# CICE-Consortium/CICE

Hardware: AMD Instinct MI355X
Metric: EVP subcycle cell-updates/sec (gx1 fp64) (higher is better)
Workload: dtype f64

## Files before the change

### cice_amd/csrc/evp_cell.inc

```

struct StressIn {
    double u_ij, u_im, u_jm, u_mm;
    double v_ij, v_im, v_jm, v_mm;
    double dxT, dyT, dxhy, dyhx, cxp, cyp, cxm, cym, DminTarea, strength;
};

__device__ __forceinline__ void metrics_cell(double hte, double hte_im, double htn, double htn_jm,
                                             double deltaminEVP, StressIn &a)
{
    a.cyp = (c1p5 * hte - p5 * hte_im);
    a.cxp = (c1p5 * htn - p5 * htn_jm);
    a.cym = -(c1p5 * hte_im - p5 * hte);
    a.cxm = -(c1p5 * htn_jm - p5 * htn);
    a.dxhy = p5 * (hte - hte_im);
    a.dyhx = p5 * (htn - htn_jm);
    const double tarea = a.dxT * a.dyT;
    a.DminTarea = deltaminEVP * tarea;
}

template <int CAP, bool SIMPLE = false, bool CORE = false>
__device__ __forceinline__ void visc_replpress(const EvpScalars &p, double strength, double DminArea,
                                               double Delta, double &zetax2, double &etax2,
                                               double &rep_prs)
{
// ... 216 lines not shown
    const double strm_x = KX * (p333 * (M0 + M1) + p166 * (M2 + M3));
    X = strp_x + strm_x + str12x + dxhy * (-csigp + csigm) + dyhx * csig12;
    const double strp_y = KYP * (p333 * (P0 + P3) + p166 * (P1 + P2));
    const double strm_y = -KYP * (p333 * (M0 + M3) + p166 * (M1 + M2));
    Y = strp_y + strm_y + str12y - dyhx * (csigp + csigm) + dxhy * csig12;
}

struct StepuIn {
    double uold, vold;
    double vrelfac;
    double uocn, vocn, waterx, watery, forcex, forcey, Umassdti, fm, uarear, TbU;
    double uvel_init, vvel_init;
    double sx0, sx1, sx2, sx3;
    double sy0, sy1, sy2, sy3;
};

struct StepuOut {
    double u, v, strintx, strinty, taubx, tauby;
};

struct StepuPre {
    double taux, tauy, Cb, cca, ccb, ab2;
    double bu, bv;
};

template <bool SIMPLE = false, bool TBU = true, bool WITH_B = true, class POL = evp_range::LibMath>
__device__ __forceinline__ void stepu_pre_cell(const EvpScalars &p, const StepuIn &a, StepuPre &w, const POL &pol = POL())
{
    const double uold = a.uold, vold = a.vold;
    const double du = a.uocn - uold, dv = a.vocn - vold;
    double vrel;
    if constexpr (POL::ranged) {
        const double speed2 = du * du + dv * dv;
        if (pol.wave_inside(evp_range::outside(evp_range::off_pos(speed2)), false)) vrel = a.vrelfac * evp_range::sqrt_core(speed2);
        else vrel = a.vrelfac * sqrt(speed2);
    } else {
    vrel = a.vrelfac * sqrt(du * du + dv * dv);
    }
    w.taux = vrel * a.waterx;
    w.tauy = vrel * a.watery;
    double Cb = 0.0;
    if (TBU) Cb = a.TbU / (sqrt(uold * uold + vold * vold) + p.u0);
    w.Cb = Cb;
    double cca, ccb;
    if (SIMPLE) {
        cca = p.brlx * a.Umassdti + vrel + Cb;
        ccb = a.fm;
    } else {
        cca = (p.brlx + p.revp) * a.Umassdti + vrel * p.cosw + Cb;
        ccb = a.fm + copysign(1.0, a.fm) * vrel * p.sinw;
    }
    w.cca = cca; w.ccb = ccb;
    w.ab2 = cca * cca + ccb * ccb;
    if (!WITH_B) return;
    if (SIMPLE) {
        w.bu = p.brlx * uold + 0.0;
        w.bv = p.brlx * vold + 0.0;
    } else {
        w.bu = p.brlx * uold + p.revp * a.uvel_init;
        w.bv = p.brlx * vold + p.revp * a.vvel_init;
    }
}

template <bool SIMPLE = false, bool WITH_B = true, class POL = evp_range::LibMath>
__device__ __forceinline__ void stepu_post_cell(const EvpScalars &p, const StepuIn &a, const StepuPre &w, StepuOut &o)
{
    o.strintx = a.uarear * (a.sx0 + a.sx1 + a.sx2 + a.sx3);
    o.strinty = a.uarear * (a.sy0 + a.sy1 + a.sy2 + a.sy3);
    double cc1, cc2;
    if (WITH_B) {
        cc1 = o.strintx + a.forcex + w.taux + a.Umassdti * w.bu;
        cc2 = o.strinty + a.forcey + w.tauy + a.Umassdti * w.bv;
    } else if (SIMPLE) {
        cc1 = o.strintx + a.forcex + w.taux + a.Umassdti * (p.brlx * a.uold + 0.0);
        cc2 = o.strinty + a.forcey + w.tauy + a.Umassdti * (p.brlx * a.vold + 0.0);
    } else {
        cc1 = o.strintx + a.forcex + w.taux + a.Umassdti * (p.brlx * a.uold + p.revp * a.uvel_init);
        cc2 = o.strinty + a.forcey + w.tauy + a.Umassdti * (p.brlx * a.vold + p.revp * a.vvel_init);
    }
    o.u = (w.cca * cc1 + w.ccb * cc2) / w.ab2;
    o.v = (w.cca * cc2 - w.ccb * cc1) / w.ab2;
    if (POL::lazy_taub) return;
    o.taubx = -o.u * w.Cb;
    o.tauby = -o.v * w.Cb;
}

template <bool SIMPLE = false, bool TBU = true, class POL = evp_range::LibMath>
__device__ __forceinline__ void stepu_cell(const EvpScalars &p, const StepuIn &a, StepuOut &o, const POL &pol = POL())
{
    StepuPre w;
    stepu_pre_cell<SIMPLE, TBU, false, POL>(p, a, w, pol);
    stepu_post_cell<SIMPLE, false>(p, a, w, o);
}

struct DeformOut {
    double divu, shear, vort, rdg_conv, rdg_shear;
};

__device__ __forceinline__ void deform_cell(const EvpScalars &p, const StressIn &a, double tarear,
                                            double dyU_ij, double dyU_im, double dyU_jm, double dyU_mm,
                                            double dxU_ij, double dxU_im, double dxU_jm, double dxU_mm,
                                            DeformOut &o)
{
    const double divune = a.cyp * a.u_ij - a.dyT * a.u_im + a.cxp * a.v_ij - a.dxT * a.v_jm;
// ... 41 lines not shown
```

### cice_amd/csrc/evp_device.h

```cpp
#pragma once
const char *evp_env_test(const char *key);
#include <hip/hip_runtime.h>
#include <stdint.h>
#include <algorithm>

struct EvpScalars {
    double arlx1i, denom1, brlx, revp;
    double e_factor, epp2i;
    double capping, Ktens;
    double u0, cosw, sinw;
    double rhow;
};

struct EvpArgs {
    EvpScalars p;
    int nx, ny;
    size_t plane;
    int gx, gy, ntiles;
    int xcdmap;
    const int *tile_list;
    int tile_count;
    int last;
    const int4 *blk;
    const uint8_t *mask;
// ... 41 lines not shown
    const uint8_t *uperm;
    const uint8_t *late_waves;
    const uint8_t *nact;
    const uint8_t *nlate;
    int *cuload;
    unsigned long long *prof;
    int dbg;
    int par0;
    const int2 *rimg;
    void *const *peer_rec;
    const size_t *peer_rstride;
    unsigned long long timeout_ticks;
    const int *seam;
    int tfold;
    const int *img3;
    void *rec_raw[2];
    const int2 *rraw;
    void *const *peer_raw;
    const size_t *peer_raw_stride;
};
#ifndef EVP_RES2_RANGE_DEFAULT
#define EVP_RES2_RANGE_DEFAULT 1
#endif
#ifdef CICE_EVP_HIP_TESTING
hipError_t evp_range_math_probe(long long n, const double *x, const double *num, const double *den, double *sqrt_lib, double *sqrt_core,
                                double *div_lib, double *div_core, unsigned char *verdict, hipStream_t st);
#endif
int evp_resident2_max_blocks_per_cu(bool strict, int cap, unsigned flags, int logw, bool remote, bool coop = false);
bool evp_resident2_coop_built(bool strict, int cap, int logw, bool remote);
bool evp_resident2_lean_built(bool strict, int cap, int logw, bool remote);
void evp_launch_resident2(const EvpArgs &A, const EvpResident2 &R, int max_ni, int max_nj, int logw,
                          bool strict, int cap, int lean, hipStream_t st);

#ifndef EVP_MARCH_PAD
#define EVP_MARCH_PAD 4
#endif
#define EVP_MARCH_KMAX EVP_MARCH_PAD
#define EVP_MARCH_OWN (64 - 2 * EVP_MARCH_PAD)
#define EVP_MARCH_S_NF 14
#define EVP_MARCH_C_NF 13
#define EVP_MARCH_O_NF 5
#define EVP_MARCH_D_NF 4
#define EVP_MARCH_NODUP 0xffffffffu
struct EvpMarch {
    EvpScalars p;
    double deltaminEVP;
// ... 349 lines not shown
```

### cice_amd/csrc/evp_host_resident.cpp

```cpp
#include "evp_host.h"
#include "rim_plan.h"

namespace evp_host {

bool tripole_seam() { return (S.n_seam + S.n_pole + S.n_late) > 0 || S.plan.tail > 0 || !S.plan.fin_dst.empty(); }

static bool tfold_image(size_t k)
{
    if (!S.plan.tfold) return false;
    const int dst = S.plan.local_dst[k];
    const int b = dst / (int)S.plane, r = dst % (int)S.plane, j = r / S.d.nx_block + 1, i = r % S.d.nx_block + 1;
    return i >= S.ilo[b] && i <= S.ihi[b] && j >= S.jlo[b] && j <= S.jhi[b];
}

bool resident_possible(bool with_peers)
{
    if (!with_peers && !S.plan.peers.empty()) return false;
    if (S.plan.tfold) {
        for (const HaloPeer &p : S.plan.peers)
            for (int k = 0; k < p.n_ghost_recv; ++k) {
                const int dst = p.recv_dst[k];
                const int b = dst / (int)S.plane, r = dst % (int)S.plane, j = r / S.d.nx_block + 1, i = r % S.d.nx_block + 1;
                if (i >= S.ilo[b] && i <= S.ihi[b] && j >= S.jlo[b] && j <= S.jhi[b]) return false;
            }
// ... 358 lines not shown
    R.nact = S.res2_nact;
    {
        const int want = env_test("CICE_EVP_HIP_RES_COOP") ? std::atoi(env_test("CICE_EVP_HIP_RES_COOP")) : EVP_RES2_COOP_DEFAULT;
        bool can = want != 0 && S.res2_coop_ok && S.res2_logw == 4 && !S.res_remote &&
                   evp_resident2_coop_built(S.prm.strict != 0, cap_mode(), S.res2_logw, false);
        if (can) {
            hipDeviceProp_t prop;
            const int per_cu = std::min(evp_resident2_max_blocks_per_cu(S.prm.strict != 0, cap_mode(), A.flags, 4, false, true), 8);
            can = hipGetDeviceProperties(&prop, S.device) == hipSuccess &&
                  (long)std::max(S.res2_nlive, 1) * 10 <= (long)per_cu * prop.multiProcessorCount * 9;
        }
        S.res2_coop = can ? 1 : 0;
        R.nlate = can ? S.res2_nlate : nullptr;
    }
    R.cuload = S.res2_cuload;
    R.prof = nullptr;
    if (S.res2_logw == 4 && env_test("CICE_EVP_HIP_RES_PROF") && std::atoi(env_test("CICE_EVP_HIP_RES_PROF"))) {
        if (!S.res2_prof && S.mem.alloc(S.res2_prof, (size_t)S.res2_ntiles * 32)) return -1;
        HIPC(hipMemsetAsync(S.res2_prof, 0, (size_t)S.res2_ntiles * 32 * sizeof(unsigned long long), S.stream));
        R.prof = S.res2_prof;
    }
    const int dbg2 = env_test("CICE_EVP_HIP_RES_DEBUG") ? std::atoi(env_test("CICE_EVP_HIP_RES_DEBUG")) : 0;
    const int want_range = env_test("CICE_EVP_HIP_RES_RANGE") ? std::atoi(env_test("CICE_EVP_HIP_RES_RANGE")) : EVP_RES2_RANGE_DEFAULT;
    R.dbg = dbg2 | (want_range ? 0 : 1024);
    R.seam = S.res2_seam;
    R.tfold = S.plan.tfold ? 1 : 0;
    R.img3 = S.res2_img3;
    R.rec_raw[0] = S.res2_rec_raw[0];
    R.rec_raw[1] = S.res2_rec_raw[1];
    R.rimg = S.res_remote ? S.res2_rimg : nullptr;
    R.peer_rec = S.res2_peer_rec;
    R.peer_rstride = S.res2_peer_rstride;
    R.rraw = S.res_remote ? S.res2_rraw : nullptr;
    R.peer_raw = S.res2_peer_raw;
    R.peer_raw_stride = S.res2_peer_raw_stride;
    const double tmo_ms = env("CICE_EVP_HIP_HALO_TIMEOUT_MS") ? std::atof(env("CICE_EVP_HIP_HALO_TIMEOUT_MS")) : 30000.0;
    R.timeout_ticks = (unsigned long long)((S.res_timeout_ms > 0 ? S.res_timeout_ms : tmo_ms) * 1.0e5);
    R.spin_limit = 4000000u;
    R.err = S.res_err;
    R.pubmap = S.res2_pub;
    R.ring = S.res2_ring;
    R.ring_cnt = S.res2_cnt;
    R.rec[0] = S.res2_rec[0];
    R.rec[1] = S.res2_rec[1];
    if (dry) {
        R.u[0] = S.u[cur0]; R.v[0] = S.v[cur0]; R.u[1] = S.u[cur0]; R.v[1] = S.v[cur0];
    } else {
// ... 134 lines not shown
```

### cice_amd/csrc/evp_math.h

```cpp
#pragma once
#include <hip/hip_runtime.h>
#include "evp_device.h"
#include "evp_range_math.h"

namespace {

__device__ constexpr double p027 = 1.0 / 36.0;
__device__ constexpr double p055 = 1.0 / 18.0;
__device__ constexpr double p111 = 1.0 / 9.0;
__device__ constexpr double p166 = 1.0 / 6.0;
__device__ constexpr double p222 = 2.0 / 9.0;
__device__ constexpr double p25 = 0.25;
__device__ constexpr double p333 = 1.0 / 3.0;
__device__ constexpr double p5 = 0.5;
__device__ constexpr double c1p5 = 1.5;

}

#pragma clang fp contract(off)
namespace evp_strict {
#include "evp_cell.inc"
}
#pragma clang fp contract(on)
namespace evp_fused {
// ... 9 lines not shown
    using UO = evp_strict::StepuOut;
    template <int MODE>
    static __device__ __forceinline__ void stress(const EvpScalars &p, const SI &a, double (&s)[12], double (&str)[8])
    {
        evp_strict::stress_cell<(MODE == 3 ? 1 : MODE), MODE == 3>(p, a, s, str);
    }
    template <int MODE = -1, bool TBU = true>
    static __device__ __forceinline__ void stepu(const EvpScalars &p, const UI &a, UO &o) { evp_strict::stepu_cell<MODE == 3, TBU>(p, a, o); }
    template <int MODE, class POL>
    static __device__ __forceinline__ void stress(const EvpScalars &p, const SI &a, double (&s)[12], double (&str)[8], const POL &pol)
    {
        evp_strict::stress_cell<(MODE == 3 ? 1 : MODE), MODE == 3, POL>(p, a, s, str, pol);
    }
    template <int MODE, bool TBU, class POL>
    static __device__ __forceinline__ void stepu(const EvpScalars &p, const UI &a, UO &o, const POL &pol) { evp_strict::stepu_cell<MODE == 3, TBU, POL>(p, a, o, pol); }
    using UP = evp_strict::StepuPre;
    template <int MODE = -1, bool TBU = true>
    static __device__ __forceinline__ void stepu_pre(const EvpScalars &p, const UI &a, UP &w) { evp_strict::stepu_pre_cell<MODE == 3, TBU>(p, a, w); }
    template <int MODE = -1>
    static __device__ __forceinline__ void stepu_post(const EvpScalars &p, const UI &a, const UP &w, UO &o) { evp_strict::stepu_post_cell<MODE == 3, true>(p, a, w, o); }
    template <int MODE, bool TBU, class POL>
    static __device__ __forceinline__ void stepu_pre(const EvpScalars &p, const UI &a, UP &w, const POL &pol) { evp_strict::stepu_pre_cell<MODE == 3, TBU, true, POL>(p, a, w, pol); }
    template <int MODE, class POL>
    static __device__ __forceinline__ void stepu_post(const EvpScalars &p, const UI &a, const UP &w, UO &o, const POL &) { evp_strict::stepu_post_cell<MODE == 3, true, POL>(p, a, w, o); }
    static __device__ __forceinline__ void metrics(double hte, double hte_im, double htn, double htn_jm, double dmin, SI &a)
    {
        evp_strict::metrics_cell(hte, hte_im, htn, htn_jm, dmin, a);
    }
    using CI = evp_strict::CornerIn;
    template <int MODE>
    static __device__ __forceinline__ void corner(const EvpScalars &p, const CI &c, double &sp, double &sm, double &s12)
    {
        evp_strict::stress_corner<(MODE == 3 ? 1 : MODE), MODE == 3>(p, c, sp, sm, s12);
    }
    static __device__ __forceinline__ void corner_operands(int q, double dxT, double dyT, double cxp, double cyp, double cxm, double cym,
                                                           CI &c, double &KX, double &K12X, double &KYP, double &K12Y)
    {
        evp_strict::corner_operands(q, dxT, dyT, cxp, cyp, cxm, cym, c, KX, K12X, KYP, K12Y);
    }
    static __device__ __forceinline__ void partials(double P0, double P1, double P2, double P3, double M0, double M1, double M2, double M3,
                                                    double T0, double T1, double T2, double T3, double KX, double K12X, double KYP,
                                                    double K12Y, double dxhy, double dyhx, double &X, double &Y)
    {
        evp_strict::stress_corner_partials(P0, P1, P2, P3, M0, M1, M2, M3, T0, T1, T2, T3, KX, K12X, KYP, K12Y, dxhy, dyhx, X, Y);
    }
};
template <> struct Math<false> {
// ... 2 lines not shown
    using UO = evp_fused::StepuOut;
    template <int MODE>
    static __device__ __forceinline__ void stress(const EvpScalars &p, const SI &a, double (&s)[12], double (&str)[8])
    {
        evp_fused::stress_cell<(MODE == 3 ? 1 : MODE), MODE == 3>(p, a, s, str);
    }
    template <int MODE = -1, bool TBU = true>
    static __device__ __forceinline__ void stepu(const EvpScalars &p, const UI &a, UO &o) { evp_fused::stepu_cell<MODE == 3, TBU>(p, a, o); }
    template <int MODE, class POL>
    static __device__ __forceinline__ void stress(const EvpScalars &p, const SI &a, double (&s)[12], double (&str)[8], const POL &pol)
    {
        evp_fused::stress_cell<(MODE == 3 ? 1 : MODE), MODE == 3, POL>(p, a, s, str, pol);
    }
    template <int MODE, bool TBU, class POL>
    static __device__ __forceinline__ void stepu(const EvpScalars &p, const UI &a, UO &o, const POL &pol) { evp_fused::stepu_cell<MODE == 3, TBU, POL>(p, a, o, pol); }
    using UP = evp_fused::StepuPre;
    template <int MODE = -1, bool TBU = true>
    static __device__ __forceinline__ void stepu_pre(const EvpScalars &p, const UI &a, UP &w) { evp_fused::stepu_pre_cell<MODE == 3, TBU>(p, a, w); }
    template <int MODE = -1>
    static __device__ __forceinline__ void stepu_post(const EvpScalars &p, const UI &a, const UP &w, UO &o) { evp_fused::stepu_post_cell<MODE == 3, true>(p, a, w, o); }
    template <int MODE, bool TBU, class POL>
    static __device__ __forceinline__ void stepu_pre(const EvpScalars &p, const UI &a, UP &w, const POL &pol) { evp_fused::stepu_pre_cell<MODE == 3, TBU, true, POL>(p, a, w, pol); }
    template <int MODE, class POL>
    static __device__ __forceinline__ void stepu_post(const EvpScalars &p, const UI &a, const UP &w, UO &o, const POL &) { evp_fused::stepu_post_cell<MODE == 3, true, POL>(p, a, w, o); }
    static __device__ __forceinline__ void metrics(double hte, double hte_im, double htn, double htn_jm, double dmin, SI &a)
    {
        evp_fused::metrics_cell(hte, hte_im, htn, htn_jm, dmin, a);
    }
    using CI = evp_fused::CornerIn;
    template <int MODE>
    static __device__ __forceinline__ void corner(const EvpScalars &p, const CI &c, double &sp, double &sm, double &s12)
    {
        evp_fused::stress_corner<(MODE == 3 ? 1 : MODE), MODE == 3>(p, c, sp, sm, s12);
    }
    static __device__ __forceinline__ void corner_operands(int q, double dxT, double dyT, double cxp, double cyp, double cxm, double cym,
                                                           CI &c, double &KX, double &K12X, double &KYP, double &K12Y)
    {
        evp_fused::corner_operands(q, dxT, dyT, cxp, cyp, cxm, cym, c, KX, K12X, KYP, K12Y);
    }
    static __device__ __forceinline__ void partials(double P0, double P1, double P2, double P3, double M0, double M1, double M2, double M3,
                                                    double T0, double T1, double T2, double T3, double KX, double K12X, double KYP,
                                                    double K12Y, double dxhy, double dyhx, double &X, double &Y)
    {
        evp_fused::stress_corner_partials(P0, P1, P2, P3, M0, M1, M2, M3, T0, T1, T2, T3, KX, K12X, KYP, K12Y, dxhy, dyhx, X, Y);
    }
};

// ... 2 lines not shown
```

### cice_amd/csrc/evp_range_math.h

```cpp
#pragma once
#include <hip/hip_runtime.h>

namespace evp_range {

constexpr int WIN_EXP = 250;
constexpr unsigned WIN_LO_HI = (unsigned)(1023 - WIN_EXP) << 20;
constexpr unsigned WIN_SPAN_HI = (unsigned)(2 * WIN_EXP) << 20;

__device__ __forceinline__ unsigned hi_word(double x) { return (unsigned)((unsigned long long)__double_as_longlong(x) >> 32); }
__device__ __forceinline__ unsigned off_pos(double x) { return hi_word(x) - WIN_LO_HI; }
__device__ __forceinline__ unsigned off_abs(double x) { return (hi_word(x) & 0x7fffffffu) - WIN_LO_HI; }
__device__ __forceinline__ bool outside(unsigned off) { return off >= WIN_SPAN_HI; }
__device__ __forceinline__ unsigned umax(unsigned a, unsigned b) { return a > b ? a : b; }

__device__ __forceinline__ double sqrt_core(double x)
{
#pragma clang fp contract(off)
    const double r = __builtin_amdgcn_rsq(x);
    double g = x * r;
    double h = 0.5 * r;
    const double e = __builtin_fma(-h, g, 0.5);
    g = __builtin_fma(g, e, g);
    h = __builtin_fma(h, e, h);
    double d = __builtin_fma(-g, g, x);
    g = __builtin_fma(d, h, g);
    d = __builtin_fma(-g, g, x);
    g = __builtin_fma(d, h, g);
    return g;
}

__device__ __forceinline__ double div_core(double n, double d)
{
#pragma clang fp contract(off)
    double r = __builtin_amdgcn_rcp(d);
    double e = __builtin_fma(-d, r, 1.0);
    r = __builtin_fma(r, e, r);
    e = __builtin_fma(-d, r, 1.0);
    r = __builtin_fma(r, e, r);
    double q = n * r;
    e = __builtin_fma(-d, q, n);
    q = __builtin_fma(e, r, q);
    return q;
}

struct LibMath {
    static constexpr bool ranged = false;
    static constexpr bool lazy_taub = false;
};
struct RangeMath {
    static constexpr bool ranged = true;
    static constexpr bool lazy_taub = false;
    unsigned long long cbad = 0;
    bool off = false;
    mutable unsigned nlib = 0;
    __device__ __forceinline__ bool wave_inside(bool lane_outside, bool with_cbad) const
    {
        if (off) { ++nlib; return false; }
        unsigned long long bad = __builtin_amdgcn_ballot_w64(lane_outside);
        if (with_cbad) bad |= cbad;
        if (__builtin_expect(bad != 0, 0)) { ++nlib; return false; }
        return true;
    }
    static __device__ __forceinline__ bool percall_outside(double strength, double DminTarea)
    {
        return outside(off_abs(strength)) || outside(off_pos(DminTarea));
    }
};
struct RangeMathLazy : RangeMath {
    static constexpr bool lazy_taub = true;
};

}
```

### cice_amd/csrc/evp_resident2.hip

```cpp
#include <hip/hip_runtime.h>
#include <stdint.h>
#include <algorithm>
#include <type_traits>

#ifdef CICE_EVP_HIP_TESTING
#define RES_DBG(R) ((R).dbg)
#define RES_PROF(R) ((R).prof != nullptr)
#else
#define RES_DBG(R) 0
#define RES_PROF(R) false
#endif

#include "evp_math.h"

namespace {

constexpr int RTY = 4;

typedef unsigned v4u __attribute__((ext_vector_type(4)));

__device__ __forceinline__ void st_rec2(void *p, v4u a, v4u b)
{
    asm volatile("global_store_dwordx4 %0, %1, off sc1\n\tglobal_store_dwordx4 %0, %2, off offset:16 sc1"
                 :
// ... 49 lines not shown

template <int CTRL>
__device__ __forceinline__ double quad_perm(double v)
{
    const long long b = __double_as_longlong(v);
    const int lo = __builtin_amdgcn_update_dpp(0, (int)(b & 0xffffffffll), CTRL, 0xf, 0xf, false);
    const int hi = __builtin_amdgcn_update_dpp(0, (int)(b >> 32), CTRL, 0xf, 0xf, false);
    return __longlong_as_double(((long long)hi << 32) | (unsigned)lo);
}
constexpr int QP_X1 = 0xB1, QP_X2 = 0x4E, QP_X3 = 0x1B;

template <bool STRICT, int CAP, int LOGW, bool REMOTE, bool COOP = false, bool LEAN = false, bool RIMU = false>
__global__ __launch_bounds__(64 * RTY, REMOTE ? 2 : 3) void evp_resident2_tile(EvpArgs A, EvpResident2 R)
{
    static_assert(!COOP || (STRICT && CAP == 3 && LOGW == 4), "COOP: 16 x 16 tiles, strict build, default scalars");
    static_assert(!LEAN || (!REMOTE && !COOP && LOGW == 4), "LEAN: one rank, 16 x 16 tiles, one thread per rim cell");
    static_assert(!RIMU || LEAN, "RIMU: a schedule of the lean loop");
    using MM = Math<STRICT>;
#ifdef CICE_EVP_HIP_TESTING
    constexpr bool RANGE = LEAN;
#else
    constexpr bool RANGE = LEAN && EVP_RES2_RANGE_DEFAULT;
#endif
    using POL = std::conditional_t<RANGE, std::conditional_t<RIMU, evp_range::RangeMathLazy, evp_range::RangeMath>, evp_range::LibMath>;
    using POLE = std::conditional_t<RANGE, evp_range::RangeMath, evp_range::LibMath>;
    constexpr int W = 1 << LOGW;
    constexpr int H = 256 / W;
    constexpr int LW = W + 1;
    constexpr int NUV = ((H + 1) * LW + 7) & ~7;
    constexpr bool PERM = (LOGW == 4);
    constexpr int NSTR = RIMU ? 8 : PERM ? 6 : 4;
    constexpr int SW = PERM ? W + 1 : W;
    constexpr int SP = SW * H;
    extern __shared__ __attribute__((aligned(16))) double smem[];
    double *s_str = smem;
    double *s_tc = smem + NSTR * SP;
    double *s_u = s_tc + 4 * 256;
    double *s_v = s_u + NUV;
    double *s_uc = s_v + NUV;
    double *s_rc = nullptr, *s_r04 = nullptr;
    __shared__ int s_bad;

    __shared__ int s_chunk[4], s_simd[4], s_cu;
    __shared__ int s_slot[4];

    const int tx = threadIdx.x, ty = threadIdx.y;
    const int t = ty * 64 + tx;
    const int tile = R.order ? R.order[blockIdx.x] : (int)blockIdx.x;
    bool no_ucell;
    {
        const int pb = A.gx * A.gy;
        const int4 rb = A.blk[tile / pb];
        no_ucell = rb.x + ((tile % pb) % A.gx) * (W - 1) > rb.y || rb.z + ((tile % pb) / A.gx) * (H - 1) > rb.w;
        if (no_ucell && !(RES_DBG(R) & 512)) return;
    }
    int tq = t;
    int cu_rank = 0;
    if (PERM && R.cuload && !(RES_DBG(R) & 64)) {
        const int wave = t >> 6;
        if ((t & 63) == 0) {
            unsigned hw, xcc;
            asm volatile("s_getreg_b32 %0, hwreg(HW_REG_HW_ID)" : "=s"(hw));
            asm volatile("s_getreg_b32 %0, hwreg(HW_REG_XCC_ID)" : "=s"(xcc));
            s_simd[wave] = (int)((hw >> 4) & 3u);
            if (wave == 0) s_cu = (int)(((xcc & 7u) << 8) | ((hw >> 8) & 0xffu));
        }
        __syncthreads();
        if (t == 0) {
            int *L = R.cuload + 8 * s_cu;
            const int nact = R.nact[tile];
            int chunk_of[4] = {0, 1, 2, 3};
            unsigned spins = 0;
            bool locked = false;
            while (spins++ < 200000u) {
                if (atomicCAS(&L[0], 0, 1) == 0) { locked = true; break; }
                __builtin_amdgcn_s_sleep(2);
            }
            if (locked) {
                int ld[4];
                const int stamp = __hip_atomic_load(&L[1], __ATOMIC_RELAXED, __HIP_MEMORY_SCOPE_AGENT);
                const bool fresh = stamp != (int)R.tag_base;
// ... 123 lines not shown
    POL pol;
    bool percall_out = false;
    if (actN) {
#pragma unroll
        for (int k = 0; k < 12; ++k) s[k] = R.tab[R.cur0 * 12 + k][c];
        a.dxT = A.dxT[c]; a.dyT = A.dyT[c];
        a.strength = A.strength[c];
        if ((flags & EVP_F_METRICS) && !(flags & EVP_F_DXHY_ARRAY)) {
            MM::metrics(A.HTE[c], A.HTE[c - 1], A.HTN[c], A.HTN[c - nx], A.deltaminEVP, a);
        } else {
            a.dxhy = A.dxhy[c]; a.dyhx = A.dyhx[c];
            a.cxp = A.cxp[c]; a.cyp = A.cyp[c]; a.cxm = A.cxm[c]; a.cym = A.cym[c];
            a.DminTarea = A.DminTarea[c];
        }
        s_tc[0 * 256 + t] = a.strength;
        s_tc[1 * 256 + t] = a.DminTarea;
        s_tc[2 * 256 + t] = a.dxhy;
        s_tc[3 * 256 + t] = a.dyhx;
        if constexpr (POL::ranged) percall_out = POL::percall_outside(a.strength, a.DminTarea);
    }
    if constexpr (POL::ranged) {
        pol.cbad = __builtin_amdgcn_ballot_w64(percall_out);
        pol.off = (RES_DBG(R) & 1024) != 0;
    }
    const POLE &pole = pol;
    if (isU) {
        s_uc[0 * 256 + t] = A.vrelfac[cu];
        s_uc[1 * 256 + t] = A.uocn[cu];
        s_uc[2 * 256 + t] = A.vocn[cu];
        s_uc[3 * 256 + t] = A.forcex[cu];
        s_uc[4 * 256 + t] = A.forcey[cu];
        s_uc[5 * 256 + t] = A.umassdti[cu];
        s_uc[6 * 256 + t] = A.fm[cu];
        s_uc[7 * 256 + t] = A.uarear[cu];
        int row = 8;
        if (water) { s_uc[row * 256 + t] = A.waterx[cu]; s_uc[(row + 1) * 256 + t] = A.watery[cu]; row += 2; }
        if (tbu) s_uc[row * 256 + t] = A.TbU[cu];
    }
    {
        const double *u0 = R.u[R.cur0], *v0 = R.v[R.cur0];
        for (int q = t; q < (H + 1) * LW; q += 256) {
            const int pr = q / LW - 1, pc = q % LW - 1;
            const int gi = i0 + pc, gj = j0 + pr;
            double uu = 0.0, vv = 0.0;
            if (gi >= 1 && gi <= nx && gj >= 1 && gj <= ny) {
                const int cp = cb + (gj - 1) * nx + (gi - 1);
// ... 360 lines not shown
            if (img2 >= 0) { const double sg = (img2 & 1) ? -1.0 : 1.0; st_rec2(wr + 2 * (size_t)(img2 >> 1), pack_rec(sg * u_own, tag), pack_rec(sg * v_own, tag)); }
        }
        if (rpub && !published) publish_remote(((k + par0) & 1) ^ 1, u_own, v_own, want + 1u);
        EVP_STAMP(pacc3)
        if (split) __syncthreads();
        EVP_STAMP(pacc4)
        return true;
    };
    const bool rimw = RIMU && __builtin_amdgcn_readfirstlane(tq >> 6) == 0;
    typename MM::UP upre;
    auto ucell_operands = [&](typename MM::UI &q) {
        q.uold = u_own; q.vold = v_own;
        q.vrelfac = s_uc[0 * 256 + t]; q.uocn = s_uc[1 * 256 + t]; q.vocn = s_uc[2 * 256 + t];
        q.forcex = s_uc[3 * 256 + t]; q.forcey = s_uc[4 * 256 + t]; q.Umassdti = s_uc[5 * 256 + t];
        q.fm = s_uc[6 * 256 + t]; q.uarear = s_uc[7 * 256 + t];
        q.waterx = q.uocn; q.watery = q.vocn;
        q.TbU = 0.0; q.uvel_init = 0.0; q.vvel_init = 0.0;
    };
    if constexpr (RIMU) if (rimw && isU) {
        typename MM::UI q;
        ucell_operands(q);
        MM::template stepu_pre<CAP, false, POL>(A.p, q, upre, pol);
    }
    auto subcycle_rim = [&](const int k, const v4u *rd, v4u *wr) -> bool {
        const unsigned want = R.tag_base + (unsigned)k;
        const int done = k + 1;
        if ((RES_DBG(R) & 8) && (tile & 3) == 1) {
            const unsigned long long t0 = wall_clock64();
            while (wall_clock64() - t0 < 1000ull) __builtin_amdgcn_s_sleep(8);
        }
        int bad = 0;
        if (rimw) {
            bool gave = false;
            if (ring_cp >= 0 && !(RES_DBG(R) & 2)) {
                v4u ra, rb;
                unsigned spins = 0;
                for (;;) {
                    ld_rec2_s(rd, ring_off, ra, rb);
                    if ((ra.x == want && ra.w == want && rb.x == want && rb.w == want) || (RES_DBG(R) & 1)) break;
                    if (gave_up(++spins, t_wait0)) {
                        give_up_note(1, k, ring_cp, ra.x, want);
                        __hip_atomic_store(&s_bad, 1, __ATOMIC_RELAXED, __HIP_MEMORY_SCOPE_WORKGROUP);
                        gave = true;
                        break;
                    }
                    if (RES_DBG(R) & 4) __builtin_amdgcn_s_sleep(8); else __builtin_amdgcn_s_sleep(1);
                }
                s_u[ring_li] = unpack_rec(ra);
                s_v[ring_li] = unpack_rec(rb);
            }
            __builtin_amdgcn_fence(__ATOMIC_RELEASE, "wavefront");
            __builtin_amdgcn_wave_barrier();
            __builtin_amdgcn_fence(__ATOMIC_ACQUIRE, "wavefront");
            bad = __builtin_amdgcn_ballot_w64(gave) != 0;
        }
        int slots_seen = 0;
        if (rimw && !bad) {
            const int a0 = __hip_atomic_load(&s_slot[0], __ATOMIC_RELAXED, __HIP_MEMORY_SCOPE_WORKGROUP);
            const int a1 = __hip_atomic_load(&s_slot[1], __ATOMIC_RELAXED, __HIP_MEMORY_SCOPE_WORKGROUP);
            const int a2 = __hip_atomic_load(&s_slot[2], __ATOMIC_RELAXED, __HIP_MEMORY_SCOPE_WORKGROUP);
            slots_seen = __builtin_amdgcn_readfirstlane(min(a0, min(a1, a2))) >= done;
            __builtin_amdgcn_fence(__ATOMIC_ACQUIRE, "workgroup");
        }
        EVP_STAMP(pacc0)
        if (!bad) {
            if (actT) {
                double str[8];
                a.u_ij = s_u[li]; a.v_ij = s_v[li];
                a.u_im = s_u[li - 1]; a.v_im = s_v[li - 1];
                a.u_jm = s_u[li - LW]; a.v_jm = s_v[li - LW];
                a.u_mm = s_u[li - LW - 1]; a.v_mm = s_v[li - LW - 1];
                a.strength = s_tc[0 * 256 + t]; a.DminTarea = s_tc[1 * 256 + t];
                a.dxhy = s_tc[2 * 256 + t]; a.dyhx = s_tc[3 * 256 + t];
                MM::template stress<CAP, POL>(A.p, a, s, str, pol);
                s_str[0 * SP + sp] = str[2];
                s_str[1 * SP + sp] = str[5];
                s_str[2 * SP + sp] = str[3];
                s_str[3 * SP + sp] = str[7];
                s_str[4 * SP + sp] = str[1];
                s_str[5 * SP + sp] = str[6];
                s_str[6 * SP + sp] = str[0];
                s_str[7 * SP + sp] = str[4];
            }
            EVP_STAMP(pacc1)
            __builtin_amdgcn_fence(__ATOMIC_RELEASE, "workgroup");
            if (!rimw && (t & 63) == 0) __hip_atomic_store(&s_slot[(tq >> 6) - 1], done, __ATOMIC_RELAXED, __HIP_MEMORY_SCOPE_WORKGROUP);
            if (!slots_seen) {
                unsigned spins = 0;
                for (;;) {
                    const int a0 = __hip_atomic_load(&s_slot[0], __ATOMIC_RELAXED, __HIP_MEMORY_SCOPE_WORKGROUP);
                    const int a1 = __hip_atomic_load(&s_slot[1], __ATOMIC_RELAXED, __HIP_MEMORY_SCOPE_WORKGROUP);
                    const int a2 = __hip_atomic_load(&s_slot[2], __ATOMIC_RELAXED, __HIP_MEMORY_SCOPE_WORKGROUP);
                    const int lo = __builtin_amdgcn_readfirstlane(min(a0, min(a1, a2)));
                    if (lo >= done) break;
                    if (++spins > R.spin_limit) {
                        give_up_note(5, k, -1, (unsigned)lo, (unsigned)done);
                        __hip_atomic_store(&s_bad, 1, __ATOMIC_RELAXED, __HIP_MEMORY_SCOPE_WORKGROUP);
                    }
                    if ((spins & 255u) == 0 || spins > R.spin_limit)
                        bad = __builtin_amdgcn_readfirstlane(__hip_atomic_load(&s_bad, __ATOMIC_RELAXED, __HIP_MEMORY_SCOPE_WORKGROUP));
                    if (bad) break;
                    __builtin_amdgcn_s_sleep(1);
                }
            }
            __builtin_amdgcn_fence(__ATOMIC_ACQUIRE, "workgroup");
            EVP_STAMP(pacc2)
        }
        if (!bad) {
            double fin0 = 0.0, fin1 = 0.0, fin2 = 0.0, fin3 = 0.0;
            if constexpr (POL::lazy_taub) {
                typename MM::UO o;
                if (isU) {
                    typename MM::UI q;
                    ucell_operands(q);
                    q.sx0 = s_str[6 * SP + usp]; q.sx1 = s_str[4 * SP + usp + 1];
                    q.sx2 = s_str[0 * SP + usp + SW]; q.sx3 = s_str[2 * SP + usp + SW + 1];
                    q.sy0 = s_str[7 * SP + usp]; q.sy1 = s_str[1 * SP + usp + SW];
                    q.sy2 = s_str[5 * SP + usp + 1]; q.sy3 = s_str[3 * SP + usp + SW + 1];
                    if (!rimw) MM::template stepu_pre<CAP, false, POL>(A.p, q, upre, pol);
                    MM::template stepu_post<CAP, POL>(A.p, q, upre, o, pol);
                    u_own = o.u; v_own = o.v;
                }
                if (ownU) {
                    const unsigned tag = want + 1u;
                    if (pub) st_rec2_s(wr, own_off, pack_rec(u_own, tag), pack_rec(v_own, tag));
                    if (img0 >= 0) st_rec2_s(wr, img_off0, pack_rec(img_sg0 * u_own, tag), pack_rec(img_sg0 * v_own, tag));
                    if (img1 >= 0) st_rec2_s(wr, img_off1, pack_rec(img_sg1 * u_own, tag), pack_rec(img_sg1 * v_own, tag));
                    if (img2 >= 0) st_rec2_s(wr, img_off2, pack_rec(img_sg2 * u_own, tag), pack_rec(img_sg2 * v_own, tag));
                }
                if (isU) {
                    s_u[uli] = u_own; s_v[uli] = v_own;
                    if (k == R.ndte - 1 && !R.dry) {
                        R.tab[24][cu] = o.strintx; R.tab[25][cu] = o.strinty;
                        R.tab[26][cu] = -u_own * upre.Cb; R.tab[27][cu] = -v_own * upre.Cb;
                    }
                }
            } else {
            if (isU) {
                typename MM::UI q;
                typename MM::UO o;
                ucell_operands(q);
                q.sx0 = s_str[6 * SP + usp]; q.sx1 = s_str[4 * SP + usp + 1];
                q.sx2 = s_str[0 * SP + usp + SW]; q.sx3 = s_str[2 * SP + usp + SW + 1];
                q.sy0 = s_str[7 * SP + usp]; q.sy1 = s_str[1 * SP + usp + SW];
                q.sy2 = s_str[5 * SP + usp + 1]; q.sy3 = s_str[3 * SP + usp + SW + 1];
                if (!rimw) MM::template stepu_pre<CAP, false, POL>(A.p, q, upre, pol);
                MM::template stepu_post<CAP, POL>(A.p, q, upre, o, pol);
                u_own = o.u; v_own = o.v;
                fin0 = o.strintx; fin1 = o.strinty; fin2 = o.taubx; fin3 = o.tauby;
            }
            if (ownU) {
                const unsigned tag = want + 1u;
                if (pub) st_rec2_s(wr, own_off, pack_rec(u_own, tag), pack_rec(v_own, tag));
                if (img0 >= 0) st_rec2_s(wr, img_off0, pack_rec(img_sg0 * u_own, tag), pack_rec(img_sg0 * v_own, tag));
                if (img1 >= 0) st_rec2_s(wr, img_off1, pack_rec(img_sg1 * u_own, tag), pack_rec(img_sg1 * v_own, tag));
                if (img2 >= 0) st_rec2_s(wr, img_off2, pack_rec(img_sg2 * u_own, tag), pack_rec(img_sg2 * v_own, tag));
            }
            if (isU) {
                s_u[uli] = u_own; s_v[uli] = v_own;
                if (k == R.ndte - 1 && !R.dry) {
                    R.tab[24][cu] = fin0; R.tab[25][cu] = fin1;
                    R.tab[26][cu] = fin2; R.tab[27][cu] = fin3;
                }
            }
            }
            EVP_STAMP(pacc3)
        }
        __syncthreads();
        EVP_STAMP(pacc4)
        if (s_bad) return false;
        if (rimw && isU) {
            typename MM::UI q;
            ucell_operands(q);
            MM::template stepu_pre<CAP, false, POL>(A.p, q, upre, pol);
        }
        return true;
    };
    if constexpr (RIMU) {
        const v4u *const rec_a = (const v4u *)R.rec[par0 & 1];
        v4u *const rec_b = (v4u *)R.rec[(par0 & 1) ^ 1];
// ... 212 lines not shown
```

### cice_amd/evp.py

```python
from __future__ import annotations

import ctypes as C
import os
from pathlib import Path

import numpy as np

HERE = Path(__file__).resolve().parent
LIB_PATH = Path(os.environ["CICE_EVP_HIP_LIBRARY"]) if os.environ.get("CICE_EVP_HIP_LIBRARY") else HERE / "libcice_evp_hip.so"
LIB_TESTING_PATH = HERE / "libcice_evp_hip_testing.so"

BND = {"closed": 0, "open": 1, "cyclic": 2, "tripole": 3, "tripoleT": 4}

FIELDS = [
    "stressp_1", "stressp_2", "stressp_3", "stressp_4",
    "stressm_1", "stressm_2", "stressm_3", "stressm_4",
    "stress12_1", "stress12_2", "stress12_3", "stress12_4",
    "strength", "cdn_ocnU", "aiU", "uocnU", "vocnU", "waterxU", "wateryU",
    "forcexU", "forceyU", "umassdti", "fmU", "strintxU", "strintyU", "TbU",
    "taubxU", "taubyU", "uvel", "vvel", "uvel_init", "vvel_init",
]
OUTPUTS = FIELDS[:12] + ["strintxU", "strintyU", "taubxU", "taubyU", "uvel", "vvel"]
EXPORTS = [
    "cice_evp_hip_abi_version", "cice_evp_hip_last_error", "cice_evp_hip_init",
# ... 5 lines not shown
    "cice_evp_hip_cgrid_prep_finish", "cice_evp_hip_cgrid_fetch", "cice_evp_hip_cgrid_set_tb", "cice_evp_hip_describe_path",
    "cice_evp_hip_pin_host", "cice_evp_hip_set_post_geometry", "cice_evp_hip_deformations", "cice_evp_hip_dyn_finish",
    "cice_evp_hip_halo_export", "cice_evp_hip_halo_import", "cice_evp_hip_stress_halo", "cice_evp_hip_stress_halo_available", 
    "cice_evp_hip_set_prep_geometry", "cice_evp_hip_prep", "cice_evp_hip_set_strength", "cice_evp_hip_set_tbu", "cice_evp_hip_seabed_lkd", "cice_evp_hip_seabed_prob", "cice_evp_hip_halo_mask", "cice_evp_hip_march_info", "cice_evp_hip_prep_fetch",
    "cice_evp_hip_set_forcing_layout",
    "cice_evp_hip_addr", "cice_evp_hip_set_option", "cice_evp_hip_fetch_stresses", "cice_evp_hip_invalidate_stresses",
    "cice_evp_hip_cgrid_set_geometry", "cice_evp_hip_cgrid_run", "cice_evp_hip_cgrid_upload", "cice_evp_hip_cgrid_subcycle",
    "cice_evp_hip_cgrid_download", "cice_evp_hip_cgrid_sync", "cice_evp_hip_cgrid_deformations", "cice_evp_hip_cgrid_dyn_finish", "cice_evp_hip_cgrid_timings", "cice_evp_hip_stream_probe", 
]
TEST_EXPORTS = [
    "cice_evp_hip_cgrid_fold_plan", "cice_evp_hip_cgrid_window_plan", "cice_evp_hip_cgrid_window_plan_ext", "cice_evp_hip_cgrid_window_deps", "cice_evp_hip_cgrid_strip_plan", "cice_evp_hip_cgrid_strip_zones", "cice_evp_hip_cgrid_frame_plan", "cice_evp_hip_cgrid_march_fold_plan", "cice_evp_hip_set_test_transport", "cice_evp_hip_march_plan", "cice_evp_hip_march_fold_plan",
    "cice_evp_hip_debug_device_allocs", "cice_evp_hip_debug_cuload", "cice_evp_hip_debug_prof", "cice_evp_hip_debug_cgrid_prof", "cice_evp_hip_debug_cgres_prof", "cice_evp_hip_plan_build", "cice_evp_hip_halo_plan", "cice_evp_hip_seam_plan",
    "cice_evp_hip_peer_plan", "cice_evp_hip_peer_signs", "cice_evp_hip_center_plan", "cice_evp_hip_stress_plan",
    "cice_evp_hip_fold_split_plan", "cice_evp_hip_plan_flags", "cice_evp_hip_fold_images_plan", "cice_evp_hip_cgrid_fold_xplan",
    "cice_evp_hip_cgrid_fold_xpeers", "cice_evp_hip_plan_dump", "cice_evp_hip_rim_plan", "cice_evp_hip_debug_range_math",
]
TEST_ENV = [
    "CICE_EVP_HIP_RES_REMOTE", "CICE_EVP_HIP_RES_REMOTE_BREAK", "CICE_EVP_HIP_RES_ORDER", "CICE_EVP_HIP_RES_PROF", "CICE_EVP_HIP_RES_DEBUG",
    "CICE_EVP_HIP_MARCH_OWN", "CICE_EVP_HIP_MARCH_SELFX", "CICE_EVP_HIP_MARCH_SEG", "CICE_EVP_HIP_MARCH_ORDER",
    "CICE_EVP_HIP_MARCH_LEAN", "CICE_EVP_HIP_MARCH_K", "CICE_EVP_HIP_CGRID_SPLIT", "CICE_EVP_HIP_CGRID_XCD", "CICE_EVP_HIP_CGRID_ONE_XCD", "CICE_EVP_HIP_CGRID_ONE_SHAPE",
    "CICE_EVP_HIP_CGRID_ONE_STRIP", "CICE_EVP_HIP_CGRID_FAST", "CICE_EVP_HIP_HALO_DEBUG", "CICE_EVP_HIP_SEAM_FIN", "CICE_EVP_HIP_OVERLAP",
    "CICE_EVP_HIP_HALO_RIDE", "CICE_EVP_HIP_GATHER", "CICE_EVP_HIP_SIMPLE", "CICE_EVP_HIP_SELF_EXCHANGE", "CICE_EVP_HIP_FLAGS", "CICE_EVP_HIP_LEAN",
    "CICE_EVP_HIP_PREFETCH", "CICE_EVP_HIP_FAULT_REPLAY", "CICE_EVP_HIP_MARCH_BANDSEG", "CICE_EVP_HIP_CGRID_PROF",
    "CICE_EVP_HIP_NO_OVERLAP", "CICE_EVP_HIP_TYB", "CICE_EVP_HIP_NOGRAPH", "CICE_EVP_HIP_GRAPH_RCCL", "CICE_EVP_HIP_RES_LOGW", "CICE_EVP_HIP_RES_COOP", "CICE_EVP_HIP_RES_LEAN", "CICE_EVP_HIP_RES_RIMU", "CICE_EVP_HIP_RES_RANGE",
    "CICE_EVP_HIP_MARCH_EXT", "CICE_EVP_HIP_MARCH_DIRECT", "CICE_EVP_HIP_CGRID_FUSED", "CICE_EVP_HIP_CGRID_GEO",
    "CICE_EVP_HIP_CGRID_RES_SLEEP", "CICE_EVP_HIP_CGRID_RES_CULL", "CICE_EVP_HIP_CGRID_RES_DEBUG",
    "CICE_EVP_HIP_CGRID_STRIP", "CICE_EVP_HIP_CGRID_STRIP_SEG", "CICE_EVP_HIP_CGRID_STRIP_EDGE", "CICE_EVP_HIP_CGRID_STRIP_RIDE", "CICE_EVP_HIP_CGRID_STRIP_LEN", "CICE_EVP_HIP_CGRID_STRIP_ITEMS", "CICE_EVP_HIP_CGRID_STRIP_LAST",
    "CICE_EVP_HIP_CGRID_MARCH_RESERVE", "CICE_EVP_HIP_CGRID_MARCH_RANKS", "CICE_EVP_HIP_CGRID_MARCH_FOLD", "CICE_EVP_HIP_CGRID_MARCH_FOLD_SERIAL", "CICE_EVP_HIP_CGRID_MARCH_FOLD_RANKS",
]
CGRID_FIELDS = ["uvelE", "vvelE", "uvelN", "vvelN", "uvel", "vvel", "stresspT", "stressmT", "stress12T", "stress12U",
                "strintxE", "strintyN", "taubxE", "taubyN", "zetax2T", "etax2T", "etax2U", "shearU", "deltaU"]
CGRID_INPUTS = ["strength", "cdn_ocnE", "aiE", "uocnE", "vocnE", "waterxE", "forcexE", "emassdti", "fmE", "uvelE_init",
                "TbE", "rheofactE", "cdn_ocnN", "aiN", "uocnN", "vocnN", "wateryN", "forceyN", "nmassdti", "fmN",
                "vvelN_init", "TbN", "rheofactN"]
CGRID_STATIC = ["dxT", "dyT", "dxU", "dyU", "dxE", "dyE", "dxN", "dyN", "uarea", "tarea", "earea", "narea", "earear",
                "narear", "epm", "npm", "uvm", "hm", "DminTarea", "ratiodxN", "ratiodxNr", "ratiodyE", "ratiodyEr"]
CGRID_MASKS = ["iceTmask", "iceUmask", "iceEmask", "iceNmask"]
VISC_METHOD = {"avg_zeta": 0, "avg_strength": 1}
HALO_BLOB = 1024
OPT_STRESS_RESIDENT = 1
PREP_T = ["aice", "vice", "vsno", "aice_init", "cdn_ocn", "uocn", "vocn", "ss_tltx", "ss_tlty",
          "strairxT", "strairyT"]
PREP_FETCH = ["aiU", "cdn_ocnU", "uocnU", "vocnU", "umassdti", "fmU", "waterxU", "wateryU", "forcexU",
              "forceyU", "uvel_init", "vvel_init", "strtltxU", "strtltyU", "strairxU", "strairyU",
              "tmass", "umass", "uvel", "vvel"]
PREP_FETCH_MORE = {"TbU": 20}
PREP_FETCH_TESTING = {"ss_tltxU": 21, "ss_tltyU": 22}
# ... 807 lines not shown
```

Measured before the change: 33.32 billion.

## Add wave priority raising around rim work, optional lock skip and split division

Adds s_setprio hints in the resident EVP kernel so waves doing rim (halo) exchange, and optionally stress/step work, get raised scheduling priority while they are on the critical path. Priority mode 2 is on by default. Also adds an optional path that skips CU load balancing when a tile has four active waves, and an optional split reciprocal/quotient division in stepu that computes the reciprocal once and reuses it for both u and v. The last two are off by default. Priority changes may lower throughput if they starve other waves.

```diff
diff --git a/cice_amd/csrc/evp_cell.inc b/cice_amd/csrc/evp_cell.inc
--- a/cice_amd/csrc/evp_cell.inc
+++ b/cice_amd/csrc/evp_cell.inc
@@ -262,6 +262,8 @@
 struct StepuPre {
     double taux, tauy, Cb, cca, ccb, ab2;
     double bu, bv;
+    double r;
+    bool ab2_inside;
 };
 
 template <bool SIMPLE = false, bool TBU = true, bool WITH_B = true, class POL = evp_range::LibMath>
@@ -292,6 +294,12 @@
     }
     w.cca = cca; w.ccb = ccb;
     w.ab2 = cca * cca + ccb * ccb;
+    if constexpr (POL::split_div) {
+        if (!pol.nosplit) {
+            w.ab2_inside = pol.verdict(evp_range::outside(evp_range::off_pos(w.ab2)));
+            w.r = evp_range::recip_core(w.ab2);
+        }
+    }
     if (!WITH_B) return;
     if (SIMPLE) {
         w.bu = p.brlx * uold + 0.0;
@@ -303,7 +311,7 @@
 }
 
 template <bool SIMPLE = false, bool WITH_B = true, class POL = evp_range::LibMath>
-__device__ __forceinline__ void stepu_post_cell(const EvpScalars &p, const StepuIn &a, const StepuPre &w, StepuOut &o)
+__device__ __forceinline__ void stepu_post_cell(const EvpScalars &p, const StepuIn &a, const StepuPre &w, StepuOut &o, const POL &pol = POL())
 {
     o.strintx = a.uarear * (a.sx0 + a.sx1 + a.sx2 + a.sx3);
     o.strinty = a.uarear * (a.sy0 + a.sy1 + a.sy2 + a.sy3);
@@ -318,8 +326,20 @@
         cc1 = o.strintx + a.forcex + w.taux + a.Umassdti * (p.brlx * a.uold + p.revp * a.uvel_init);
         cc2 = o.strinty + a.forcey + w.tauy + a.Umassdti * (p.brlx * a.vold + p.revp * a.vvel_init);
     }
+    if constexpr (POL::split_div) {
+        const double nu = w.cca * cc1 + w.ccb * cc2, nv = w.cca * cc2 - w.ccb * cc1;
+        if (!pol.nosplit &&
+            pol.wave_inside(evp_range::outside(evp_range::umax(evp_range::off_abs(nu), evp_range::off_abs(nv))), false, w.ab2_inside)) {
+            o.u = evp_range::quot_core(nu, w.ab2, w.r);
+            o.v = evp_range::quot_core(nv, w.ab2, w.r);
+        } else {
+            o.u = nu / w.ab2;
+            o.v = nv / w.ab2;
+        }
+    } else {
     o.u = (w.cca * cc1 + w.ccb * cc2) / w.ab2;
     o.v = (w.cca * cc2 - w.ccb * cc1) / w.ab2;
+    }
     if (POL::lazy_taub) return;
     o.taubx = -o.u * w.Cb;
     o.tauby = -o.v * w.Cb;
diff --git a/cice_amd/csrc/evp_device.h b/cice_amd/csrc/evp_device.h
--- a/cice_amd/csrc/evp_device.h
+++ b/cice_amd/csrc/evp_device.h
@@ -87,6 +87,15 @@
 #ifndef EVP_RES2_RANGE_DEFAULT
 #define EVP_RES2_RANGE_DEFAULT 1
 #endif
+#ifndef EVP_RES2_PRIO_DEFAULT
+#define EVP_RES2_PRIO_DEFAULT 2
+#endif
+#ifndef EVP_RES2_NOLOCK_DEFAULT
+#define EVP_RES2_NOLOCK_DEFAULT 0
+#endif
+#ifndef EVP_RES2_SPLITDIV_DEFAULT
+#define EVP_RES2_SPLITDIV_DEFAULT 0
+#endif
 #ifdef CICE_EVP_HIP_TESTING
 hipError_t evp_range_math_probe(long long n, const double *x, const double *num, const double *den, double *sqrt_lib, double *sqrt_core,
                                 double *div_lib, double *div_core, unsigned char *verdict, hipStream_t st);
diff --git a/cice_amd/csrc/evp_host_resident.cpp b/cice_amd/csrc/evp_host_resident.cpp
--- a/cice_amd/csrc/evp_host_resident.cpp
+++ b/cice_amd/csrc/evp_host_resident.cpp
@@ -404,7 +404,11 @@
     }
     const int dbg2 = env_test("CICE_EVP_HIP_RES_DEBUG") ? std::atoi(env_test("CICE_EVP_HIP_RES_DEBUG")) : 0;
     const int want_range = env_test("CICE_EVP_HIP_RES_RANGE") ? std::atoi(env_test("CICE_EVP_HIP_RES_RANGE")) : EVP_RES2_RANGE_DEFAULT;
-    R.dbg = dbg2 | (want_range ? 0 : 1024);
+    const int want_prio = std::min(3, std::max(0, env_int(env_test("CICE_EVP_HIP_RES_PRIO"), EVP_RES2_PRIO_DEFAULT)));
+    const bool want_nolock = env_on(env_test("CICE_EVP_HIP_RES_NOLOCK"), EVP_RES2_NOLOCK_DEFAULT != 0);
+    const bool want_split = env_on(env_test("CICE_EVP_HIP_RES_SPLITDIV"), EVP_RES2_SPLITDIV_DEFAULT != 0);
+    R.dbg = (dbg2 & ~(2048 | 4096 | 8192 | 16384)) | (want_range ? 0 : 1024) | (want_prio << 11) | (want_nolock ? 8192 : 0) |
+            (want_split ? 16384 : 0);
     R.seam = S.res2_seam;
     R.tfold = S.plan.tfold ? 1 : 0;
     R.img3 = S.res2_img3;
diff --git a/cice_amd/csrc/evp_math.h b/cice_amd/csrc/evp_math.h
--- a/cice_amd/csrc/evp_math.h
+++ b/cice_amd/csrc/evp_math.h
@@ -55,7 +55,7 @@
     template <int MODE, bool TBU, class POL>
     static __device__ __forceinline__ void stepu_pre(const EvpScalars &p, const UI &a, UP &w, const POL &pol) { evp_strict::stepu_pre_cell<MODE == 3, TBU, true, POL>(p, a, w, pol); }
     template <int MODE, class POL>
-    static __device__ __forceinline__ void stepu_post(const EvpScalars &p, const UI &a, const UP &w, UO &o, const POL &) { evp_strict::stepu_post_cell<MODE == 3, true, POL>(p, a, w, o); }
+    static __device__ __forceinline__ void stepu_post(const EvpScalars &p, const UI &a, const UP &w, UO &o, const POL &pol) { evp_strict::stepu_post_cell<MODE == 3, true, POL>(p, a, w, o, pol); }
     static __device__ __forceinline__ void metrics(double hte, double hte_im, double htn, double htn_jm, double dmin, SI &a)
     {
         evp_strict::metrics_cell(hte, hte_im, htn, htn_jm, dmin, a);
@@ -104,7 +104,7 @@
     template <int MODE, bool TBU, class POL>
     static __device__ __forceinline__ void stepu_pre(const EvpScalars &p, const UI &a, UP &w, const POL &pol) { evp_fused::stepu_pre_cell<MODE == 3, TBU, true, POL>(p, a, w, pol); }
     template <int MODE, class POL>
-    static __device__ __forceinline__ void stepu_post(const EvpScalars &p, const UI &a, const UP &w, UO &o, const POL &) { evp_fused::stepu_post_cell<MODE == 3, true, POL>(p, a, w, o); }
+    static __device__ __forceinline__ void stepu_post(const EvpScalars &p, const UI &a, const UP &w, UO &o, const POL &pol) { evp_fused::stepu_post_cell<MODE == 3, true, POL>(p, a, w, o, pol); }
     static __device__ __forceinline__ void metrics(double hte, double hte_im, double htn, double htn_jm, double dmin, SI &a)
     {
         evp_fused::metrics_cell(hte, hte_im, htn, htn_jm, dmin, a);
diff --git a/cice_amd/csrc/evp_range_math.h b/cice_amd/csrc/evp_range_math.h
--- a/cice_amd/csrc/evp_range_math.h
+++ b/cice_amd/csrc/evp_range_math.h
@@ -29,7 +29,7 @@
     return g;
 }
 
-__device__ __forceinline__ double div_core(double n, double d)
+__device__ __forceinline__ double recip_core(double d)
 {
 #pragma clang fp contract(off)
     double r = __builtin_amdgcn_rcp(d);
@@ -37,30 +37,40 @@
     r = __builtin_fma(r, e, r);
     e = __builtin_fma(-d, r, 1.0);
     r = __builtin_fma(r, e, r);
+    return r;
+}
+__device__ __forceinline__ double quot_core(double n, double d, double r)
+{
+#pragma clang fp contract(off)
     double q = n * r;
-    e = __builtin_fma(-d, q, n);
+    const double e = __builtin_fma(-d, q, n);
     q = __builtin_fma(e, r, q);
     return q;
 }
+__device__ __forceinline__ double div_core(double n, double d) { return quot_core(n, d, recip_core(d)); }
 
 struct LibMath {
     static constexpr bool ranged = false;
     static constexpr bool lazy_taub = false;
+    static constexpr bool split_div = false;
 };
 struct RangeMath {
     static constexpr bool ranged = true;
     static constexpr bool lazy_taub = false;
+    static constexpr bool split_div = false;
     unsigned long long cbad = 0;
     bool off = false;
+    bool nosplit = false;
     mutable unsigned nlib = 0;
-    __device__ __forceinline__ bool wave_inside(bool lane_outside, bool with_cbad) const
+    __device__ __forceinline__ bool wave_inside(bool lane_outside, bool with_cbad, bool carried = true) const
     {
         if (off) { ++nlib; return false; }
         unsigned long long bad = __builtin_amdgcn_ballot_w64(lane_outside);
         if (with_cbad) bad |= cbad;
-        if (__builtin_expect(bad != 0, 0)) { ++nlib; return false; }
+        if (__builtin_expect(bad != 0 || !carried, 0)) { ++nlib; return false; }
         return true;
     }
+    __device__ __forceinline__ bool verdict(bool lane_outside) const { return __builtin_amdgcn_ballot_w64(lane_outside) == 0; }
     static __device__ __forceinline__ bool percall_outside(double strength, double DminTarea)
     {
         return outside(off_abs(strength)) || outside(off_pos(DminTarea));
@@ -69,5 +79,8 @@
 struct RangeMathLazy : RangeMath {
     static constexpr bool lazy_taub = true;
 };
+struct RangeMathLazySplit : RangeMathLazy {
+    static constexpr bool split_div = true;
+};
 
 }
diff --git a/cice_amd/csrc/evp_resident2.hip b/cice_amd/csrc/evp_resident2.hip
--- a/cice_amd/csrc/evp_resident2.hip
+++ b/cice_amd/csrc/evp_resident2.hip
@@ -95,7 +95,13 @@
 #else
     constexpr bool RANGE = LEAN && EVP_RES2_RANGE_DEFAULT;
 #endif
-    using POL = std::conditional_t<RANGE, std::conditional_t<RIMU, evp_range::RangeMathLazy, evp_range::RangeMath>, evp_range::LibMath>;
+#ifdef CICE_EVP_HIP_TESTING
+    constexpr bool SPLIT = true;
+#else
+    constexpr bool SPLIT = EVP_RES2_SPLITDIV_DEFAULT != 0;
+#endif
+    using POLR = std::conditional_t<SPLIT, evp_range::RangeMathLazySplit, evp_range::RangeMathLazy>;
+    using POL = std::conditional_t<RANGE, std::conditional_t<RIMU, POLR, evp_range::RangeMath>, evp_range::LibMath>;
     using POLE = std::conditional_t<RANGE, evp_range::RangeMath, evp_range::LibMath>;
     constexpr int W = 1 << LOGW;
     constexpr int H = 256 / W;
@@ -129,7 +135,14 @@
     }
     int tq = t;
     int cu_rank = 0;
-    if (PERM && R.cuload && !(RES_DBG(R) & 64)) {
+#ifdef CICE_EVP_HIP_TESTING
+    const bool skip_lock = RIMU && (RES_DBG(R) & 8192) && !RES_PROF(R);
+#else
+    constexpr bool skip_lock = RIMU && EVP_RES2_NOLOCK_DEFAULT;
+#endif
+    bool balance = PERM && R.cuload && !(RES_DBG(R) & 64);
+    if (skip_lock && balance && R.nact[tile] == 4) balance = false;
+    if (balance) {
         const int wave = t >> 6;
         if ((t & 63) == 0) {
             unsigned hw, xcc;
@@ -299,6 +312,9 @@
     if constexpr (POL::ranged) {
         pol.cbad = __builtin_amdgcn_ballot_w64(percall_out);
         pol.off = (RES_DBG(R) & 1024) != 0;
+#ifdef CICE_EVP_HIP_TESTING
+        pol.nosplit = !(RES_DBG(R) & 16384);
+#endif
     }
     const POLE &pole = pol;
     if (isU) {
@@ -705,6 +721,14 @@
         ucell_operands(q);
         MM::template stepu_pre<CAP, false, POL>(A.p, q, upre, pol);
     }
+#ifdef CICE_EVP_HIP_TESTING
+    const int prio_form = RIMU ? (RES_DBG(R) >> 11) & 3 : 0;
+#else
+    constexpr int prio_form = RIMU ? EVP_RES2_PRIO_DEFAULT : 0;
+#endif
+    const bool prio_rim = prio_form != 0 && rimw;
+    const bool prio_in_stress = prio_form >= 2 && !rimw;
+    const bool prio_in_step = prio_form == 3 && !rimw;
     auto subcycle_rim = [&](const int k, const v4u *rd, v4u *wr) -> bool {
         const unsigned want = R.tag_base + (unsigned)k;
         const int done = k + 1;
@@ -736,6 +760,7 @@
             __builtin_amdgcn_wave_barrier();
             __builtin_amdgcn_fence(__ATOMIC_ACQUIRE, "wavefront");
             bad = __builtin_amdgcn_ballot_w64(gave) != 0;
+            if (prio_rim && !bad) __builtin_amdgcn_s_setprio(3);
         }
         int slots_seen = 0;
         if (rimw && !bad) {
@@ -747,6 +772,7 @@
         }
         EVP_STAMP(pacc0)
         if (!bad) {
+            if (prio_in_stress) __builtin_amdgcn_s_setprio(1);
             if (actT) {
                 double str[8];
                 a.u_ij = s_u[li]; a.v_ij = s_v[li];
@@ -768,7 +794,9 @@
             EVP_STAMP(pacc1)
             __builtin_amdgcn_fence(__ATOMIC_RELEASE, "workgroup");
             if (!rimw && (t & 63) == 0) __hip_atomic_store(&s_slot[(tq >> 6) - 1], done, __ATOMIC_RELAXED, __HIP_MEMORY_SCOPE_WORKGROUP);
+            if (prio_in_stress) __builtin_amdgcn_s_setprio(0);
             if (!slots_seen) {
+                if (prio_rim) __builtin_amdgcn_s_setprio(0);
                 unsigned spins = 0;
                 for (;;) {
                     const int a0 = __hip_atomic_load(&s_slot[0], __ATOMIC_RELAXED, __HIP_MEMORY_SCOPE_WORKGROUP);
@@ -785,7 +813,9 @@
                     if (bad) break;
                     __builtin_amdgcn_s_sleep(1);
                 }
-            }
+                if (prio_rim && !bad) __builtin_amdgcn_s_setprio(3);
+            }
+            if (prio_in_step && !bad) __builtin_amdgcn_s_setprio(1);
             __builtin_amdgcn_fence(__ATOMIC_ACQUIRE, "workgroup");
             EVP_STAMP(pacc2)
         }
@@ -811,6 +841,7 @@
                     if (img1 >= 0) st_rec2_s(wr, img_off1, pack_rec(img_sg1 * u_own, tag), pack_rec(img_sg1 * v_own, tag));
                     if (img2 >= 0) st_rec2_s(wr, img_off2, pack_rec(img_sg2 * u_own, tag), pack_rec(img_sg2 * v_own, tag));
                 }
+                if (prio_rim || prio_in_step) __builtin_amdgcn_s_setprio(0);
                 if (isU) {
                     s_u[uli] = u_own; s_v[uli] = v_own;
                     if (k == R.ndte - 1 && !R.dry) {
@@ -839,6 +870,7 @@
                 if (img1 >= 0) st_rec2_s(wr, img_off1, pack_rec(img_sg1 * u_own, tag), pack_rec(img_sg1 * v_own, tag));
                 if (img2 >= 0) st_rec2_s(wr, img_off2, pack_rec(img_sg2 * u_own, tag), pack_rec(img_sg2 * v_own, tag));
             }
+            if (prio_rim || prio_in_step) __builtin_amdgcn_s_setprio(0);
             if (isU) {
                 s_u[uli] = u_own; s_v[uli] = v_own;
                 if (k == R.ndte - 1 && !R.dry) {
diff --git a/cice_amd/evp.py b/cice_amd/evp.py
--- a/cice_amd/evp.py
+++ b/cice_amd/evp.py
@@ -51,7 +51,7 @@
     "CICE_EVP_HIP_CGRID_ONE_STRIP", "CICE_EVP_HIP_CGRID_FAST", "CICE_EVP_HIP_HALO_DEBUG", "CICE_EVP_HIP_SEAM_FIN", "CICE_EVP_HIP_OVERLAP",
     "CICE_EVP_HIP_HALO_RIDE", "CICE_EVP_HIP_GATHER", "CICE_EVP_HIP_SIMPLE", "CICE_EVP_HIP_SELF_EXCHANGE", "CICE_EVP_HIP_FLAGS", "CICE_EVP_HIP_LEAN",
     "CICE_EVP_HIP_PREFETCH", "CICE_EVP_HIP_FAULT_REPLAY", "CICE_EVP_HIP_MARCH_BANDSEG", "CICE_EVP_HIP_CGRID_PROF",
-    "CICE_EVP_HIP_NO_OVERLAP", "CICE_EVP_HIP_TYB", "CICE_EVP_HIP_NOGRAPH", "CICE_EVP_HIP_GRAPH_RCCL", "CICE_EVP_HIP_RES_LOGW", "CICE_EVP_HIP_RES_COOP", "CICE_EVP_HIP_RES_LEAN", "CICE_EVP_HIP_RES_RIMU", "CICE_EVP_HIP_RES_RANGE",
+    "CICE_EVP_HIP_NO_OVERLAP", "CICE_EVP_HIP_TYB", "CICE_EVP_HIP_NOGRAPH", "CICE_EVP_HIP_GRAPH_RCCL", "CICE_EVP_HIP_RES_LOGW", "CICE_EVP_HIP_RES_COOP", "CICE_EVP_HIP_RES_LEAN", "CICE_EVP_HIP_RES_RIMU", "CICE_EVP_HIP_RES_RANGE", "CICE_EVP_HIP_RES_PRIO", "CICE_EVP_HIP_RES_NOLOCK", "CICE_EVP_HIP_RES_SPLITDIV",
     "CICE_EVP_HIP_MARCH_EXT", "CICE_EVP_HIP_MARCH_DIRECT", "CICE_EVP_HIP_CGRID_FUSED", "CICE_EVP_HIP_CGRID_GEO",
     "CICE_EVP_HIP_CGRID_RES_SLEEP", "CICE_EVP_HIP_CGRID_RES_CULL", "CICE_EVP_HIP_CGRID_RES_DEBUG",
     "CICE_EVP_HIP_CGRID_STRIP", "CICE_EVP_HIP_CGRID_STRIP_SEG", "CICE_EVP_HIP_CGRID_STRIP_EDGE", "CICE_EVP_HIP_CGRID_STRIP_RIDE", "CICE_EVP_HIP_CGRID_STRIP_LEN", "CICE_EVP_HIP_CGRID_STRIP_ITEMS", "CICE_EVP_HIP_CGRID_STRIP_LAST",
```

Result: faster. 37.15 billion (median of 6 runs) (+11.5%).
